# pomonam/LearnablePoolingMethods

Measured on AMD Instinct MI355X. Metric: clips/sec training step, NetVladV1 K=256 300-frame 1152-d, bs=80, 1/2/4/8 GPU, higher is better.
Workload: dtype f32

## Files before the change

### learnablepoolingmethods_amd/csrc/mha_x3.hip

```cpp
#include "lpm_common.h"
#include "operand_format.h"
#include <atomic>
#include <cstdlib>

namespace lpm {

constexpr float MX_LOG2E = 1.4426950408889634f;
constexpr float MX_LN2 = 0.6931471805599453f;
typedef __bf16 mx_bf16x8 __attribute__((ext_vector_type(8)));
typedef __bf16 mx_bf16x2 __attribute__((ext_vector_type(2)));
typedef float mx_f32x2 __attribute__((ext_vector_type(2)));
typedef unsigned mx_u32x4 __attribute__((ext_vector_type(4)));

__device__ __forceinline__ f32x4 mx_mfma(mx_u32x4 a, mx_u32x4 b, f32x4 c) {
    return __builtin_amdgcn_mfma_f32_16x16x32_bf16(__builtin_bit_cast(mx_bf16x8, a), __builtin_bit_cast(mx_bf16x8, b), c, 0, 0, 0);
}
__device__ __forceinline__ void mx_split2(float a, float b, unsigned& hi, unsigned& lo) {
    const mx_f32x2 v = {a, b};
    const mx_bf16x2 h = __builtin_convertvector(v, mx_bf16x2);
    const mx_f32x2 hf = __builtin_convertvector(h, mx_f32x2);
    const mx_bf16x2 l = __builtin_convertvector(v - hf, mx_bf16x2);
    hi = __builtin_bit_cast(unsigned, h);
    lo = __builtin_bit_cast(unsigned, l);
}
// ... 102 lines not shown
        hi[i] = h;
        lo[i] = l;
    }
}
__device__ __forceinline__ void mx_pow2_scale(float amax, float& s, float& inv) {
    const int e = (int)((__float_as_uint(amax) >> 23) & 0xffu);
    const int se = e == 0 ? 127 : min(max(258 - e, 1), 253);
    s = __uint_as_float((unsigned)se << 23);
    inv = __uint_as_float((unsigned)(254 - se) << 23);
}
template <int D>
__device__ __forceinline__ void mx_stage_transposed_h(unsigned char* dst, const float* __restrict__ src, int64_t ld, int b, int L, int LP,
                                                      int hh, int tid, int nt) {
    constexpr int NH = D / 8;
    const int TS = LP * 2 + 16;
    for (int i = tid; i < L * NH; i += nt) {
        const int row = i / NH, hf = i % NH;
        const float* p = src + ((int64_t)b * L + row) * ld + hh * D + 8 * hf;
        const float4 a = *reinterpret_cast<const float4*>(p), c = *reinterpret_cast<const float4*>(p + 4);
        const float v[8] = {a.x, a.y, a.z, a.w, c.x, c.y, c.z, c.w};
        mx_u32x4 hi, lo;
        mx_split8_h(v, 1.f, hi, lo);
        const int pos = (row & ~31) | (((row >> 2) & 3) << 3) | (((row >> 4) & 1) << 2) | (row & 3);
#pragma unroll
        for (int e = 0; e < 8; ++e) {
            const int dd = 8 * hf + e;
            *reinterpret_cast<unsigned short*>(dst + dd * TS + pos * 2) = (unsigned short)(hi[e >> 1] >> ((e & 1) * 16));
            *reinterpret_cast<unsigned short*>(dst + 16 * TS + dd * TS + pos * 2) = (unsigned short)(lo[e >> 1] >> ((e & 1) * 16));
        }
    }
}

__device__ __forceinline__ int mx_perm(int i) { return (i & ~31) | (((i >> 2) & 3) << 3) | (((i >> 4) & 1) << 2) | (i & 3); }

__host__ __device__ constexpr int mx_rowplanes_bytes(int LP, int D) { return (D / 8) * 2 * LP * 16; }
__host__ __device__ constexpr int mx_tstride(int LP) { return LP * 2 + 16; }
__host__ __device__ constexpr int mx_tplanes_bytes(int LP) { return 2 * 16 * mx_tstride(LP); }

template <int D>
__device__ __forceinline__ void mx_stage_rows(unsigned char* dst, const float* __restrict__ src, int64_t ld, int b, int L, int LP,
                                              int hh, float mul, int tid, int nt = 256) {
    constexpr int NH = D / 8;
    for (int i = tid; i < L * NH; i += nt) {
        const int row = i / NH, hf = i % NH;
        const float* p = src + ((int64_t)b * L + row) * ld + hh * D + 8 * hf;
        const float4 a = *reinterpret_cast<const float4*>(p), c = *reinterpret_cast<const float4*>(p + 4);
        const float v[8] = {a.x * mul, a.y * mul, a.z * mul, a.w * mul, c.x * mul, c.y * mul, c.z * mul, c.w * mul};
        mx_u32x4 hi, lo;
        mx_split8(v, hi, lo);
        *reinterpret_cast<mx_u32x4*>(dst + ((0 * NH + hf) * LP + row) * 16) = hi;
        *reinterpret_cast<mx_u32x4*>(dst + ((1 * NH + hf) * LP + row) * 16) = lo;
    }
}
template <int D>
__device__ __forceinline__ void mx_stage_transposed(unsigned char* dst, const float* __restrict__ src, int64_t ld, int b, int L,
                                                    int LP, int hh, int tid, int nt = 256) {
    constexpr int NH = D / 8;
    const int TS = mx_tstride(LP);
    for (int i = tid; i < L * NH; i += nt) {
        const int row = i / NH, hf = i % NH;
        const float* p = src + ((int64_t)b * L + row) * ld + hh * D + 8 * hf;
        const float4 a = *reinterpret_cast<const float4*>(p), c = *reinterpret_cast<const float4*>(p + 4);
        const float v[8] = {a.x, a.y, a.z, a.w, c.x, c.y, c.z, c.w};
        mx_u32x4 hi, lo;
        mx_split8(v, hi, lo);
        const int pos = mx_perm(row);
#pragma unroll
        for (int e = 0; e < 8; ++e) {
            const int dd = 8 * hf + e;
            const unsigned short h16 = (unsigned short)(hi[e >> 1] >> ((e & 1) * 16)), l16 = (unsigned short)(lo[e >> 1] >> ((e & 1) * 16));
            *reinterpret_cast<unsigned short*>(dst + dd * TS + pos * 2) = h16;
            *reinterpret_cast<unsigned short*>(dst + 16 * TS + dd * TS + pos * 2) = l16;
        }
    }
}

template <int D>
__device__ __forceinline__ mx_u32x4 mx_row_frag(const unsigned char* planes, int LP, int t, int l15, int g) {
    const int arr = (D == 16) ? g : ((g == 1) ? 1 : 0);
    return *reinterpret_cast<const mx_u32x4*>(planes + (arr * LP + t * 16 + l15) * 16);
}
template <int D>
__device__ __forceinline__ void mx_col_frags(const mx_u32x4& hi, const mx_u32x4& lo, int g, mx_u32x4& b1, mx_u32x4& b2) {
    const mx_u32x4 z = {0u, 0u, 0u, 0u};
    if (D == 16) {
        b1 = hi;
        b2 = (g < 2) ? lo : z;
    } else {
        b1 = (g < 2) ? hi : ((g == 2) ? lo : z);
        b2 = z;
    }
}

template <int NKT, bool AFFINE, int D, bool RAGGED>
__global__ __launch_bounds__(256) void mha_fwd_x3_kernel(const float* __restrict__ q, const float* __restrict__ k,
                                                         const float* __restrict__ v, int64_t ld, int L, int h, float scale,
                                                         const float* __restrict__ key_scale, const float* __restrict__ key_shift,
                                                         float* __restrict__ o, int64_t ldo, float* __restrict__ lse, int oimg, const MxImg im) {
    static_assert(NKT % 2 == 0, "key tiles come in pairs (32-deep PV reduction)");
    float vmax = 0.f;
    extern __shared__ __attribute__((aligned(16))) unsigned char smem[];
    constexpr int LP = NKT * 16;
    constexpr int NQ = (NKT + 3) / 4;
    const int nkt = (L + 15) >> 4;
    const float qmul = AFFINE ? scale : scale * MX_LOG2E;
    unsigned char* Kp = smem;
    unsigned char* Vt = Kp + mx_rowplanes_bytes(LP, D);
    float* ksc = reinterpret_cast<float*>(Vt + mx_tplanes_bytes(LP));
    float* ksh = ksc + LP;
    const int tid = threadIdx.x, lane = tid & 63, wave = tid >> 6;
    const int l15 = lane & 15, g = lane >> 4;
    const int lid = xcd_remap(blockIdx.x, gridDim.x);
    const int b = lid / h, hh = lid % h;
    const int TS = mx_tstride(LP);

    if (RAGGED || D < 16) {
        for (int i = tid; i < (mx_rowplanes_bytes(LP, D) + mx_tplanes_bytes(LP)) / 16; i += 256)
            reinterpret_cast<mx_u32x4*>(smem)[i] = mx_u32x4{0u, 0u, 0u, 0u};
        __syncthreads();
    }
    if (AFFINE) {
        for (int i = tid; i < LP; i += 256) {
            ksc[i] = (i < L) ? key_scale[i] * MX_LOG2E : 1.f;
            ksh[i] = (i < L) ? key_shift[i] * MX_LOG2E : 0.f;
        }
    }
    mx_stage_rows<D>(Kp, k, ld, b, L, LP, hh, 1.f, tid);
    mx_stage_transposed<D>(Vt, v, ld, b, L, LP, hh, tid);
    __syncthreads();

#pragma unroll 1
    for (int i = 0; i < NQ; ++i) {
        const int qt = wave + 4 * i;
        if (qt >= nkt) break;
        const int qrow = qt * 16 + l15;
        mx_u32x4 qh = {0u, 0u, 0u, 0u}, ql = {0u, 0u, 0u, 0u};
        if (qrow < L) {
            const float* p = q + ((int64_t)b * L + qrow) * ld + hh * D + ((D == 16) ? 8 * (g & 1) : 0);
            const float4 a = *reinterpret_cast<const float4*>(p), c = *reinterpret_cast<const float4*>(p + 4);
            const float qv[8] = {a.x * qmul, a.y * qmul, a.z * qmul, a.w * qmul, c.x * qmul, c.y * qmul, c.z * qmul, c.w * qmul};
            mx_split8(qv, qh, ql);
        }
        mx_u32x4 b1, b2;
        mx_col_frags<D>(qh, ql, g, b1, b2);
        f32x4 p[NKT];
        float m = -INFINITY;
#pragma unroll
        for (int kt = 0; kt < NKT; ++kt) {
            f32x4 acc = {0.f, 0.f, 0.f, 0.f};
            const mx_u32x4 a = mx_row_frag<D>(Kp, LP, kt, l15, g);
            acc = mx_mfma(a, b1, acc);
            if (D == 16) acc = mx_mfma(a, b2, acc);
            if (AFFINE) {
#pragma unroll
                for (int r = 0; r < 4; ++r) acc[r] = fmaf(acc[r], ksc[kt * 16 + 4 * g + r], ksh[kt * 16 + 4 * g + r]);
            }
#pragma unroll
            for (int r = 0; r < 4; ++r) {
                if (RAGGED && kt * 16 + 4 * g + r >= L) acc[r] = -INFINITY;
                m = fmaxf(m, acc[r]);
            }
            p[kt] = acc;
        }
        m = fmaxf(m, __shfl_xor(m, 16, 64));
        m = fmaxf(m, __shfl_xor(m, 32, 64));
        float sum = 0.f;
        f32x4 oa = {0.f, 0.f, 0.f, 0.f}, ob = {0.f, 0.f, 0.f, 0.f};
#pragma unroll
        for (int j = 0; j < NKT / 2; ++j) {
            float e8[8];
#pragma unroll
            for (int r = 0; r < 4; ++r) {
                e8[r] = __builtin_amdgcn_exp2f(p[2 * j][r] - m);
                e8[4 + r] = __builtin_amdgcn_exp2f(p[2 * j + 1][r] - m);
            }
#pragma unroll
            for (int r = 0; r < 8; ++r) sum += e8[r];
            mx_u32x4 ph, pl;
            mx_split8(e8, ph, pl);
            const unsigned char* va = Vt + l15 * TS + (32 * j + 8 * g) * 2;
            const mx_u32x4 vh = *reinterpret_cast<const mx_u32x4*>(va), vl = *reinterpret_cast<const mx_u32x4*>(va + 16 * TS);
            oa = mx_mfma(vh, ph, oa);
            ob = mx_mfma(vh, pl, ob);
            oa = mx_mfma(vl, ph, oa);
        }
        sum += __shfl_xor(sum, 16, 64);
        sum += __shfl_xor(sum, 32, 64);
        const float inv = 1.f / sum;
        if (qrow < L) {
            if (4 * g < D)
                mx_store_act4(o, (int64_t)b * L + qrow, ldo, hh * D + 4 * g, oimg, (oa[0] + ob[0]) * inv, (oa[1] + ob[1]) * inv,
                              (oa[2] + ob[2]) * inv, (oa[3] + ob[3]) * inv, im, vmax);
            if (g == 0) lse[((int64_t)b * h + hh) * L + qrow] = m * MX_LN2 + __logf(sum);
        }
    }
    if (oimg) of_amax_commit(im.oamax, vmax);
}

constexpr int MX_DQ_NT = 512;
template <int NKT, bool AFFINE, int D, bool RAGGED>
__global__ __launch_bounds__(MX_DQ_NT) void mha_bwd_dq_x3_kernel(const float* __restrict__ q, const float* __restrict__ k,
                                                            const float* __restrict__ v, int64_t ld, const float* __restrict__ o,
                                                            const float* __restrict__ dout, int64_t ldo,
                                                            const float* __restrict__ lse, int L, int h, float scale,
                                                            const float* __restrict__ key_scale, const float* __restrict__ key_shift,
                                                            float* __restrict__ dq, int64_t ldd, const float* __restrict__ corr_a,
                                                            const float* __restrict__ corr_b, int img, int oimg, const MxImg im) {
    extern __shared__ __attribute__((aligned(16))) unsigned char smem[];
    float vmax = 0.f;
    constexpr int LP = NKT * 16;
    const int nkt = (L + 15) >> 4;
    const float qmul = AFFINE ? scale : scale * MX_LOG2E;
    unsigned char* Kp = smem;
    unsigned char* Vp = Kp + mx_rowplanes_bytes(LP, D);
    unsigned char* Kt = Vp + mx_rowplanes_bytes(LP, D);
    float* ksc = reinterpret_cast<float*>(Kt + mx_tplanes_bytes(LP));
    float* ksh = ksc + LP;
    float* cas = ksh + LP;
    float* cbs = cas + LP;
    const int tid = threadIdx.x, lane = tid & 63, wave = tid >> 6;
    const int l15 = lane & 15, g = lane >> 4;
    const int lid = xcd_remap(blockIdx.x, gridDim.x);
    const int b = lid / h, hh = lid % h;
    const int TS = mx_tstride(LP);

    if (RAGGED || D < 16) {
        for (int i = tid; i < (2 * mx_rowplanes_bytes(LP, D) + mx_tplanes_bytes(LP)) / 16; i += MX_DQ_NT)
            reinterpret_cast<mx_u32x4*>(smem)[i] = mx_u32x4{0u, 0u, 0u, 0u};
        __syncthreads();
    }
    if (AFFINE) {
        for (int i = tid; i < LP; i += MX_DQ_NT) {
            ksc[i] = (i < L) ? key_scale[i] : 1.f;
            ksh[i] = (i < L) ? key_shift[i] : 0.f;
            cas[i] = (corr_a && i < L) ? corr_a[i] : 0.f;
            cbs[i] = (corr_b && i < L) ? corr_b[i] : 0.f;
        }
    }
    mx_stage_rows<D>(Kp, k, ld, b, L, LP, hh, 1.f, tid, MX_DQ_NT);
    mx_stage_rows<D>(Vp, v, ld, b, L, LP, hh, 1.f, tid, MX_DQ_NT);
    mx_stage_transposed<D>(Kt, k, ld, b, L, LP, hh, tid, MX_DQ_NT);
    __syncthreads();

#pragma unroll 1
    for (int qt = wave; qt < nkt; qt += MX_DQ_NT / 64) {
        const int qrow = qt * 16 + l15;
        const bool qok = qrow < L;
        mx_u32x4 qh = {0u, 0u, 0u, 0u}, ql = qh, gh = qh, gl = qh;
        float dpart = 0.f;
        if (qok) {
            const int c0 = hh * D + ((D == 16) ? 8 * (g & 1) : 0);
            const float* qp = q + ((int64_t)b * L + qrow) * ld + c0;
            const float4 a = *reinterpret_cast<const float4*>(qp), c = *reinterpret_cast<const float4*>(qp + 4);
            const float qv[8] = {a.x * qmul, a.y * qmul, a.z * qmul, a.w * qmul, c.x * qmul, c.y * qmul, c.z * qmul, c.w * qmul};
            mx_split8(qv, qh, ql);
            const int64_t off = ((int64_t)b * L + qrow) * ldo + c0;
            const float4 ga = *reinterpret_cast<const float4*>(dout + off), gc = *reinterpret_cast<const float4*>(dout + off + 4);
            float4 oa, oc;
            mx_load_o8(o, (int64_t)b * L + qrow, ldo, c0, oimg, oa, oc, im);
            const float gv[8] = {ga.x, ga.y, ga.z, ga.w, gc.x, gc.y, gc.z, gc.w};
            mx_split8(gv, gh, gl);
            dpart = ga.x * oa.x + ga.y * oa.y + ga.z * oa.z + ga.w * oa.w + gc.x * oc.x + gc.y * oc.y + gc.z * oc.z + gc.w * oc.w;
        }
        if (D == 16) dpart += __shfl_xor(dpart, 16, 64);
        const float dqv = dpart;
        const float lq = qok ? lse[((int64_t)b * h + hh) * L + qrow] * MX_LOG2E : INFINITY;
        mx_u32x4 qb1, qb2, gb1, gb2;
        mx_col_frags<D>(qh, ql, g, qb1, qb2);
        mx_col_frags<D>(gh, gl, g, gb1, gb2);
        f32x4 dqa = {0.f, 0.f, 0.f, 0.f}, dqb = {0.f, 0.f, 0.f, 0.f};
#pragma unroll 2
        for (int j = 0; j < NKT / 2; ++j) {
            float ds8[8];
#pragma unroll
            for (int t = 0; t < 2; ++t) {
                const int kt = 2 * j + t;
                const mx_u32x4 ka = mx_row_frag<D>(Kp, LP, kt, l15, g), va = mx_row_frag<D>(Vp, LP, kt, l15, g);
                f32x4 st = {0.f, 0.f, 0.f, 0.f}, dp = {0.f, 0.f, 0.f, 0.f};
                st = mx_mfma(ka, qb1, st);
                dp = mx_mfma(va, gb1, dp);
                if (D == 16) {
                    st = mx_mfma(ka, qb2, st);
                    dp = mx_mfma(va, gb2, dp);
                }
                float z[4];
#pragma unroll
                for (int r = 0; r < 4; ++r) {
                    z[r] = st[r];
                    if (AFFINE) z[r] = fmaf(st[r], ksc[kt * 16 + 4 * g + r], ksh[kt * 16 + 4 * g + r]) * MX_LOG2E;
                }
                if (RAGGED) {
#pragma unroll
                    for (int r = 0; r < 4; ++r)
                        if (kt * 16 + 4 * g + r >= L) z[r] = -INFINITY;
                }
#pragma unroll
                for (int r = 0; r < 4; ++r) {
                    const float pr = __builtin_amdgcn_exp2f(z[r] - lq);
                    float dsv = pr * (dp[r] - dqv);
                    if (AFFINE) {
                        const int key = kt * 16 + 4 * g + r;
                        dsv = dsv * ksc[key] - cas[key] - st[r] * cbs[key];
                    }
                    ds8[4 * t + r] = dsv;
                }
            }
            mx_u32x4 dh, dl;
            mx_split8(ds8, dh, dl);
            const unsigned char* kc = Kt + l15 * TS + (32 * j + 8 * g) * 2;
            const mx_u32x4 kh = *reinterpret_cast<const mx_u32x4*>(kc), kl = *reinterpret_cast<const mx_u32x4*>(kc + 16 * TS);
            dqa = mx_mfma(kh, dh, dqa);
            dqb = mx_mfma(kh, dl, dqb);
            dqa = mx_mfma(kl, dh, dqa);
        }
        if (qok && 4 * g < D)
            mx_store_grad4(dq, ((int64_t)b * L + qrow) * ldd + hh * D + 4 * g, img, (dqa[0] + dqb[0]) * scale, (dqa[1] + dqb[1]) * scale,
                           (dqa[2] + dqb[2]) * scale, (dqa[3] + dqb[3]) * scale, im, vmax);
    }
    if (img) of_amax_commit(im.gamax, vmax);
}

#ifndef LPM_DKV_NT_LONG
#define LPM_DKV_NT_LONG 1024
#endif
__host__ __device__ constexpr int mx_dkv_nt(int nkt) { return nkt >= 20 ? LPM_DKV_NT_LONG : 512; }
template <int NKT, bool AFFINE, int D, bool CORR = true>
__global__ __launch_bounds__(mx_dkv_nt(NKT)) void mha_bwd_dkv_x3_kernel(const float* __restrict__ q, const float* __restrict__ k,
                                                             const float* __restrict__ v, int64_t ld, const float* __restrict__ o,
                                                             const float* __restrict__ dout, int64_t ldo,
                                                             const float* __restrict__ lse, int L, int h, float scale,
                                                             const float* __restrict__ key_scale, const float* __restrict__ key_shift,
                                                             float* __restrict__ dk, float* __restrict__ dv, int64_t ldd,
                                                             const float* __restrict__ corr_a, const float* __restrict__ corr_b,
                                                             float* __restrict__ dz_partial, int img, int oimg, const MxImg im) {
    extern __shared__ __attribute__((aligned(16))) unsigned char smem[];
    float vmax = 0.f;
    constexpr int LP = NKT * 16;
    constexpr int MX_DKV_NT = mx_dkv_nt(NKT);
    constexpr int NH = D / 8;
    const int nkt = (L + 15) >> 4;
    const float qmul = AFFINE ? scale : scale * MX_LOG2E;
    unsigned char* Qp = smem;
    unsigned char* Gp = Qp + mx_rowplanes_bytes(LP, D);
    unsigned char* Qt = Gp + mx_rowplanes_bytes(LP, D);
    unsigned char* Gt = Qt + mx_tplanes_bytes(LP);
    float* lses = reinterpret_cast<float*>(Gt + mx_tplanes_bytes(LP));
    float* Dq = lses + LP;
    const bool stats_only = (dk == nullptr);
    const int tid = threadIdx.x, lane = tid & 63, wave = tid >> 6;
    const int l15 = lane & 15, g = lane >> 4;
    const int lid = xcd_remap(blockIdx.x, gridDim.x);
    const int b = lid / h, hh = lid % h;
    const int TS = mx_tstride(LP);

    if (L != LP || D < 16) {
        for (int i = tid; i < (2 * mx_rowplanes_bytes(LP, D) + 2 * mx_tplanes_bytes(LP)) / 16; i += MX_DKV_NT)
            reinterpret_cast<mx_u32x4*>(smem)[i] = mx_u32x4{0u, 0u, 0u, 0u};
    }
    for (int i = tid; i < LP; i += MX_DKV_NT) {
        lses[i] = (i < L) ? lse[((int64_t)b * h + hh) * L + i] * MX_LOG2E : INFINITY;
        Dq[i] = 0.f;
    }
    __syncthreads();
    for (int i0 = 0; i0 < L * NH; i0 += MX_DKV_NT) {
        const int i = i0 + tid;
        float part = 0.f;
        int row = 0;
        if (i < L * NH) {
            row = i / NH;
            const int hf = i % NH;
            const float* qp = q + ((int64_t)b * L + row) * ld + hh * D + 8 * hf;
            const int64_t off = ((int64_t)b * L + row) * ldo + hh * D + 8 * hf;
            const float4 qa = *reinterpret_cast<const float4*>(qp), qc = *reinterpret_cast<const float4*>(qp + 4);
            const float4 ga = *reinterpret_cast<const float4*>(dout + off), gc = *reinterpret_cast<const float4*>(dout + off + 4);
            float4 oa, oc;
            mx_load_o8(o, (int64_t)b * L + row, ldo, hh * D + 8 * hf, oimg, oa, oc, im);
            part = ga.x * oa.x + ga.y * oa.y + ga.z * oa.z + ga.w * oa.w + gc.x * oc.x + gc.y * oc.y + gc.z * oc.z + gc.w * oc.w;
            const float qv[8] = {qa.x * qmul, qa.y * qmul, qa.z * qmul, qa.w * qmul, qc.x * qmul, qc.y * qmul, qc.z * qmul, qc.w * qmul};
            const float gv[8] = {ga.x, ga.y, ga.z, ga.w, gc.x, gc.y, gc.z, gc.w};
            mx_u32x4 qh, ql, gh, gl;
            mx_split8(qv, qh, ql);
            mx_split8(gv, gh, gl);
            *reinterpret_cast<mx_u32x4*>(Qp + ((0 * NH + hf) * LP + row) * 16) = qh;
            *reinterpret_cast<mx_u32x4*>(Qp + ((1 * NH + hf) * LP + row) * 16) = ql;
            *reinterpret_cast<mx_u32x4*>(Gp + ((0 * NH + hf) * LP + row) * 16) = gh;
            *reinterpret_cast<mx_u32x4*>(Gp + ((1 * NH + hf) * LP + row) * 16) = gl;
            const int pos = mx_perm(row);
#pragma unroll
            for (int e = 0; e < 8; ++e) {
                const int dd = 8 * hf + e, sh = (e & 1) * 16;
                *reinterpret_cast<unsigned short*>(Qt + dd * TS + pos * 2) = (unsigned short)(qh[e >> 1] >> sh);
                *reinterpret_cast<unsigned short*>(Qt + 16 * TS + dd * TS + pos * 2) = (unsigned short)(ql[e >> 1] >> sh);
                *reinterpret_cast<unsigned short*>(Gt + dd * TS + pos * 2) = (unsigned short)(gh[e >> 1] >> sh);
                *reinterpret_cast<unsigned short*>(Gt + 16 * TS + dd * TS + pos * 2) = (unsigned short)(gl[e >> 1] >> sh);
            }
        }
        if (NH == 2) part += __shfl_xor(part, 1, 64);
        if (i < L * NH && (i % NH) == 0) Dq[row] = part;
    }
    __syncthreads();

#pragma unroll 1
    for (int kt = wave; kt < nkt; kt += MX_DKV_NT / 64) {
        const int krow = kt * 16 + l15;
        const bool kok = krow < L;
        mx_u32x4 kh = {0u, 0u, 0u, 0u}, kl = kh, vh = kh, vl = kh;
        if (kok) {
            const int64_t off = ((int64_t)b * L + krow) * ld + hh * D + ((D == 16) ? 8 * (g & 1) : 0);
            const float4 ka = *reinterpret_cast<const float4*>(k + off), kc = *reinterpret_cast<const float4*>(k + off + 4);
            const float4 va = *reinterpret_cast<const float4*>(v + off), vc = *reinterpret_cast<const float4*>(v + off + 4);
            const float kv[8] = {ka.x, ka.y, ka.z, ka.w, kc.x, kc.y, kc.z, kc.w};
            const float vv[8] = {va.x, va.y, va.z, va.w, vc.x, vc.y, vc.z, vc.w};
            mx_split8(kv, kh, kl);
            mx_split8(vv, vh, vl);
        }
        mx_u32x4 kb1, kb2, vb1, vb2;
        mx_col_frags<D>(kh, kl, g, kb1, kb2);
        mx_col_frags<D>(vh, vl, g, vb1, vb2);
        const float sck = (key_scale && kok) ? key_scale[krow] : 1.f, shk = (key_shift && kok) ? key_shift[krow] : 0.f;
        const float cak = (corr_a && kok) ? corr_a[krow] : 0.f, cbk = (corr_b && kok) ? corr_b[krow] : 0.f;
        f32x4 dka = {0.f, 0.f, 0.f, 0.f}, dkb = dka, dva = dka, dvb = dka;
        float zs = 0.f, zq = 0.f;
#pragma unroll 2
        for (int j = 0; j < NKT / 2; ++j) {
            float p8[8], ds8[8];
#pragma unroll
            for (int t = 0; t < 2; ++t) {
                const int qt = 2 * j + t;
                const mx_u32x4 qa = mx_row_frag<D>(Qp, LP, qt, l15, g), ga = mx_row_frag<D>(Gp, LP, qt, l15, g);
                f32x4 st = {0.f, 0.f, 0.f, 0.f}, dp = {0.f, 0.f, 0.f, 0.f};
                st = mx_mfma(qa, kb1, st);
                dp = mx_mfma(ga, vb1, dp);
                if (D == 16) {
                    st = mx_mfma(qa, kb2, st);
                    dp = mx_mfma(ga, vb2, dp);
                }
                const float4 lq4v = *reinterpret_cast<const float4*>(lses + qt * 16 + 4 * g);
                const float4 dq4v = *reinterpret_cast<const float4*>(Dq + qt * 16 + 4 * g);
                const float lq4[4] = {lq4v.x, lq4v.y, lq4v.z, lq4v.w}, dq4[4] = {dq4v.x, dq4v.y, dq4v.z, dq4v.w};
#pragma unroll
                for (int r = 0; r < 4; ++r) {
                    const int qr = qt * 16 + 4 * g + r;
                    const float sraw = st[r];
                    float z = sraw;
                    if (AFFINE) z = fmaf(sraw, sck, shk) * MX_LOG2E;
                    if (!kok) z = -INFINITY;
                    const float pr = __builtin_amdgcn_exp2f(z - lq4[r]);
                    const float dz = pr * (dp[r] - dq4[r]);
                    float dsv = dz;
                    if (AFFINE) {
                        zs += dz;
                        zq = fmaf(dz, sraw, zq);
                        if constexpr (CORR) dsv = (qr < L) ? dz * sck - cak - sraw * cbk : 0.f;
                        else dsv = (qr < L) ? dz * sck : 0.f;
                    }
                    p8[4 * t + r] = pr;
                    ds8[4 * t + r] = dsv;
                }
            }
            if (!stats_only) {
                mx_u32x4 ph, pl, dh, dl;
                mx_split8(p8, ph, pl);
                mx_split8(ds8, dh, dl);
                const int offt = l15 * TS + (32 * j + 8 * g) * 2;
                const mx_u32x4 gth = *reinterpret_cast<const mx_u32x4*>(Gt + offt), gtl = *reinterpret_cast<const mx_u32x4*>(Gt + 16 * TS + offt);
                const mx_u32x4 qth = *reinterpret_cast<const mx_u32x4*>(Qt + offt), qtl = *reinterpret_cast<const mx_u32x4*>(Qt + 16 * TS + offt);
                dva = mx_mfma(gth, ph, dva);
                dvb = mx_mfma(gth, pl, dvb);
                dva = mx_mfma(gtl, ph, dva);
                dka = mx_mfma(qth, dh, dka);
                dkb = mx_mfma(qth, dl, dkb);
                dka = mx_mfma(qtl, dh, dka);
            }
        }
        if (!stats_only && kok && 4 * g < D) {
            const int64_t off = ((int64_t)b * L + krow) * ldd + hh * D + 4 * g;
            const float kmul = AFFINE ? 1.f : MX_LN2;
            mx_store_dk4(dk, (int64_t)b * L + krow, ldd, hh * D + 4 * g, img, (dka[0] + dkb[0]) * kmul, (dka[1] + dkb[1]) * kmul, (dka[2] + dkb[2]) * kmul, (dka[3] + dkb[3]) * kmul, im, vmax);
            mx_store_grad4(dv, off, img, dva[0] + dvb[0], dva[1] + dvb[1], dva[2] + dvb[2], dva[3] + dvb[3], im, vmax);
        }
        if (dz_partial) {
            zs += __shfl_xor(zs, 16, 64); zs += __shfl_xor(zs, 32, 64);
            zq += __shfl_xor(zq, 16, 64); zq += __shfl_xor(zq, 32, 64);
            if (g == 0 && kok) {
                float* out = dz_partial + ((int64_t)b * h + hh) * 2 * L;
                out[krow] = zs;
                out[L + krow] = zq;
            }
        }
    }
    if (img) of_amax_commit(im.gamax, vmax);
}

template <int NKT, bool AFFINE, int D, bool RAGGED>
__global__ __launch_bounds__(MX_DQ_NT) void mha_bwd_dq_h_kernel(const float* __restrict__ q, const float* __restrict__ k,
                                                            const float* __restrict__ v, int64_t ld, const float* __restrict__ o,
                                                            const float* __restrict__ dout, int64_t ldo,
                                                            const float* __restrict__ lse, int L, int h, float scale,
                                                            const float* __restrict__ key_scale, const float* __restrict__ key_shift,
                                                            float* __restrict__ dq, int64_t ldd, const float* __restrict__ corr_a,
                                                            const float* __restrict__ corr_b, int img, int oimg, const MxImg im) {
    extern __shared__ __attribute__((aligned(16))) unsigned char smem[];
    float vmax = 0.f;
    constexpr int LP = NKT * 16;
    constexpr int NT = MX_DQ_NT;
    const int nkt = (L + 15) >> 4;
    const float qmul = AFFINE ? scale : scale * MX_LOG2E;
    unsigned char* Kp = smem;
    unsigned char* Vp = Kp + mx_rowplanes_bytes(LP, D);
    unsigned char* Kt = Vp + mx_rowplanes_bytes(LP, D);
    float* ksc = reinterpret_cast<float*>(Kt + mx_tplanes_bytes(LP));
    float* ksh = ksc + LP;
    float* cas = ksh + LP;
    float* cbs = cas + LP;
    const int tid = threadIdx.x, lane = tid & 63, wave = tid >> 6;
    const int l15 = lane & 15, g = lane >> 4;
    const int lid = xcd_remap(blockIdx.x, gridDim.x);
    const int b = lid / h, hh = lid % h;
    const int TS = mx_tstride(LP);
// ... 359 lines not shown
    const int lid = xcd_remap(blockIdx.x, gridDim.x);
    const int b = lid / h, hh = lid % h;
    constexpr int D4 = D / 4;
    float *Qm, *Sq;
    if (moments) {
        Qm = reinterpret_cast<float*>(smem);
        Sq = Qm + D * D;
        for (int i = tid; i < D * D + D; i += 256) Qm[i] = moments[(int64_t)lid * (D * D + D) + i] * (i < D * D ? scale * scale : scale);
        __syncthreads();
    } else {
        float* qs = reinterpret_cast<float*>(smem);
        Qm = qs + (size_t)L * D;
        Sq = Qm + D * D;
        mx_q_moments<D>(q, ld, b, L, hh, scale, qs, Qm, Sq, Sq + D, tid);
    }
    const int c4 = tid % D4;
    float qm[4][D], sq4[4];
#pragma unroll
    for (int u = 0; u < 4; ++u) {
        sq4[u] = Sq[4 * c4 + u];
#pragma unroll
        for (int e = 0; e < D4; ++e) {
            const float4 t = *reinterpret_cast<const float4*>(Qm + (4 * c4 + u) * D + 4 * e);
            qm[u][4 * e] = t.x; qm[u][4 * e + 1] = t.y; qm[u][4 * e + 2] = t.z; qm[u][4 * e + 3] = t.w;
        }
    }
    for (int i = tid; i < L * D4; i += 256) {
        const int row = i / D4;
        const float* kp = k + ((int64_t)b * L + row) * ld + hh * D;
        float kv[D];
#pragma unroll
        for (int e = 0; e < D4; ++e) {
            const float4 t = *reinterpret_cast<const float4*>(kp + 4 * e);
            kv[4 * e] = t.x; kv[4 * e + 1] = t.y; kv[4 * e + 2] = t.z; kv[4 * e + 3] = t.w;
        }
        const float ca = corr_a[row], cb = corr_b[row];
        float* dp = dk + ((int64_t)b * L + row) * ldd + hh * D + 4 * c4;
        float4 g = *reinterpret_cast<float4*>(dp);
        float r[4];
#pragma unroll
        for (int u = 0; u < 4; ++u) {
            float t = 0.f;
#pragma unroll
            for (int e = 0; e < D; ++e) t = fmaf(qm[u][e], kv[e], t);
            r[u] = fmaf(cb, t, ca * sq4[u]);
        }
        g.x -= r[0]; g.y -= r[1]; g.z -= r[2]; g.w -= r[3];
        if (dk_img) mx_store_grad4(dk_img, ((int64_t)b * L + row) * ldi + hh * D + 4 * c4, img, g.x, g.y, g.z, g.w, im, vmax);
        else *reinterpret_cast<float4*>(dp) = g;
    }
    if (dk_img) of_amax_commit(im.gamax, vmax);
}

static inline size_t mx_bwd_dq_lds(int LP, int D) { return (size_t)2 * mx_rowplanes_bytes(LP, D) + mx_tplanes_bytes(LP) + 4 * LP * 4; }
static inline size_t mx_bwd_dkv_lds(int LP, int D) { return (size_t)2 * mx_rowplanes_bytes(LP, D) + 2 * mx_tplanes_bytes(LP) + 2 * LP * 4 + 16; }
static inline size_t mx_fwd_lds(int LP, int D) { return (size_t)mx_rowplanes_bytes(LP, D) + mx_tplanes_bytes(LP) + 2 * LP * 4; }

template <typename KernT>
static int mx_reserve(KernT kern, size_t bytes, const char* what) {
    if (hipFuncSetAttribute((const void*)kern, hipFuncAttributeMaxDynamicSharedMemorySize, (int)bytes) != hipSuccess) {
        (void)hipGetLastError();
        set_error("%s: cannot reserve %zu bytes of LDS", what, bytes);
        return LPM_ERR_LAUNCH;
    }
    return LPM_OK;
}

}

#define LPM_MX_CHECK(name)                                                                                        \
    LPM_REQUIRE(B > 0 && L > 0 && h > 0 && (d == 8 || d == 16) && L <= 512, LPM_ERR_UNSUPPORTED_SHAPE,              \
                name ": need d in {8,16} and L <= 512 (L=%d d=%d)", L, d);                                          \
    LPM_REQUIRE(ld >= (int64_t)h * d && ld % 4 == 0, LPM_ERR_BADARG, name ": bad leading dimension")

static std::atomic<int> g_mha_bwd_terms{lpm::env_first_is("LPM_MHA_BWD_TERMS", '2') ? 2 : 3};
extern "C" int lpm_mha_bwd_set_terms(int terms) {
    if (terms != 2 && terms != 3) return g_mha_bwd_terms.load();
    return g_mha_bwd_terms.exchange(terms);
}

static lpm::MxImg mx_img(const LpmOperandFormat* o_fmt, const LpmOperandFormat* g_fmt) {
    const lpm::OperandFmt fo = lpm::operand_fmt(o_fmt), fg = lpm::operand_fmt(g_fmt);
    return lpm::MxImg{fo.f16, fo.planes, fo.scale, 1.f / fo.scale, fo.amax, fg.f16, fg.planes, fg.scale, fg.amax, 0, 0};
}
static int mx_fwd_launch(const float* q, const float* k, const float* v, int64_t ld, int B, int L, int h, int d, float scale,
                         const float* key_scale, const float* key_shift, float* o, int64_t ldo, float* lse, int oimg,
                         lpm_stream_t stream, const char* what, const LpmOperandFormat* o_fmt = nullptr) {
    using namespace lpm;
    const MxImg im = mx_img(o_fmt, nullptr);
    hipStream_t s = (hipStream_t)stream;
    const int nkt = (L + 15) / 16;
    dim3 grid(B * h);
#define LPM_MX_FWD3(N, AFF, DD, RG)                                                                              \
    do {                                                                                                         \
        auto kern = mha_fwd_x3_kernel<N, AFF, DD, RG>;                                                           \
        const size_t lds = mx_fwd_lds(N * 16, DD);                                                               \
        if (int rc = mx_reserve(kern, lds, what)) return rc;                                                     \
        hipLaunchKernelGGL(kern, grid, dim3(256), lds, s, q, k, v, ld, L, h, scale, key_scale, key_shift, o, ldo, lse, oimg, im); \
    } while (0)
#define LPM_MX_FWD1(N, AFF, RG)        \
    do {                               \
        if (d == 16) LPM_MX_FWD3(N, AFF, 16, RG); \
        else LPM_MX_FWD3(N, AFF, 8, RG); \
    } while (0)
#define LPM_MX_FWD(N)                  \
    do {                               \
        if (key_scale) LPM_MX_FWD1(N, true, true); \
        else if (L == N * 16) LPM_MX_FWD1(N, false, false); \
        else LPM_MX_FWD1(N, false, true); \
// ... 10 lines not shown
}

extern "C" int lpm_mha_fwd_x3(const float* q, const float* k, const float* v, int64_t ld, int B, int L, int h, int d, float scale,
                              const float* key_scale, const float* key_shift, float* o, int64_t ldo, float* lse,
                              lpm_stream_t stream) {
    using namespace lpm;
    LPM_REQUIRE(q && k && v && o && lse, LPM_ERR_BADARG, "lpm_mha_fwd_x3: null pointer");
    LPM_MX_CHECK("lpm_mha_fwd_x3");
    LPM_REQUIRE((key_scale == nullptr) == (key_shift == nullptr), LPM_ERR_BADARG, "lpm_mha_fwd_x3: key_scale/key_shift go together");
    LPM_REQUIRE(ldo >= (int64_t)h * d && ldo % 4 == 0, LPM_ERR_BADARG, "lpm_mha_fwd_x3: bad ldo");
    LPM_REQUIRE((((uintptr_t)q | (uintptr_t)k | (uintptr_t)v | (uintptr_t)o) & 15) == 0, LPM_ERR_BADARG,
                "lpm_mha_fwd_x3: pointers must be 16-byte aligned");
    return mx_fwd_launch(q, k, v, ld, B, L, h, d, scale, key_scale, key_shift, o, ldo, lse, 0, stream, "lpm_mha_fwd_x3");
}

extern "C" int lpm_mha_fwd_x3_image(const float* q, const float* k, const float* v, int64_t ld, int B, int L, int h, int d,
                                    float scale, void* o3, float* lse, lpm_stream_t stream) {
    using namespace lpm;
    LPM_REQUIRE(q && k && v && o3 && lse, LPM_ERR_BADARG, "lpm_mha_fwd_x3_image: null pointer");
    LPM_MX_CHECK("lpm_mha_fwd_x3_image");
    LPM_REQUIRE((((uintptr_t)q | (uintptr_t)k | (uintptr_t)v | (uintptr_t)o3) & 15) == 0, LPM_ERR_BADARG,
                "lpm_mha_fwd_x3_image: pointers must be 16-byte aligned");
    return mx_fwd_launch(q, k, v, ld, B, L, h, d, scale, nullptr, nullptr, (float*)o3, 0, lse, h * d, stream, "lpm_mha_fwd_x3_image");
}
extern "C" int lpm_mha_fwd_x3_image_fmt(const float* q, const float* k, const float* v, int64_t ld, int B, int L, int h, int d,
                                        float scale, void* o3, float* lse, const LpmOperandFormat* o_fmt, lpm_stream_t stream) {
    using namespace lpm;
    LPM_REQUIRE(q && k && v && o3 && lse, LPM_ERR_BADARG, "lpm_mha_fwd_x3_image: null pointer");
    LPM_MX_CHECK("lpm_mha_fwd_x3_image");
    LPM_REQUIRE((((uintptr_t)q | (uintptr_t)k | (uintptr_t)v | (uintptr_t)o3) & 15) == 0, LPM_ERR_BADARG,
                "lpm_mha_fwd_x3_image: pointers must be 16-byte aligned");
    if (const int rc = operand_fmt_check(o_fmt, "lpm_mha_fwd_x3_image")) return rc;
    return mx_fwd_launch(q, k, v, ld, B, L, h, d, scale, nullptr, nullptr, (float*)o3, 0, lse, h * d, stream, "lpm_mha_fwd_x3_image", o_fmt);
}

static int mx_bwd_launch(const float* q, const float* k, const float* v, int64_t ld, const float* o, const float* dout, int64_t ldo,
                         const float* lse, int B, int L, int h, int d, float scale, const float* key_scale, const float* key_shift,
                         float* dq, float* dk, float* dv, int64_t ldd, const float* corr_a, const float* corr_b, float* dz_partial,
                         int img, int oimg, lpm_stream_t stream, const char* what, const LpmOperandFormat* o_fmt = nullptr,
                         const LpmOperandFormat* g_fmt = nullptr, int64_t dk_plain_ld = 0) {
    using namespace lpm;
    MxImg im = mx_img(o_fmt, g_fmt);
    if (dk_plain_ld) {
        im.dk_plain = 1;
        im.dk_ld = dk_plain_ld;
    }
    hipStream_t s = (hipStream_t)stream;
    const int nkt = (L + 15) / 16;
    dim3 grid(B * h);
    const bool h16 = g_mha_bwd_terms.load(std::memory_order_relaxed) == 2 && !corr_a;
#define LPM_MX_BWDH_Q(N, AFF, DD, RG)                                                                                  \
    do {                                                                                                               \
        auto kq = mha_bwd_dq_h_kernel<N, AFF, DD, RG>;                                                                 \
        const size_t lq = mx_bwd_dq_lds(N * 16, DD);                                                                   \
        if (int rc = mx_reserve(kq, lq, what)) return rc;                                                              \
        hipLaunchKernelGGL(kq, grid, dim3(MX_DQ_NT), lq, s, q, k, v, ld, o, dout, ldo, lse, L, h, scale, key_scale, key_shift, \
                           dq, ldd, corr_a, corr_b, img, oimg, im);                                                    \
    } while (0)
#define LPM_MX_BWDH_KV(N, AFF, DD)                                                                                     \
    do {                                                                                                               \
        auto kk = mha_bwd_dkv_h_kernel<N, AFF, DD, false>;                                                             \
        const size_t lk = mx_bwd_dkv_lds(N * 16, DD);                                                                  \
        if (int rc = mx_reserve(kk, lk, what)) return rc;                                                              \
        hipLaunchKernelGGL(kk, grid, dim3(mx_dkv_nt(N)), lk, s, q, k, v, ld, o, dout, ldo, lse, L, h, scale, key_scale, key_shift, \
                           dk, dv, ldd, corr_a, corr_b, dz_partial, img, oimg, im);                                    \
    } while (0)
#define LPM_MX_BWD3(N, AFF, DD, RG)                                                                                    \
    do {                                                                                                               \
        if (h16) {                                                                                                     \
            if (dq) LPM_MX_BWDH_Q(N, AFF, DD, RG);                                                                     \
            if (dk || dz_partial) LPM_MX_BWDH_KV(N, AFF, DD);                                                          \
            break;                                                                                                     \
        }                                                                                                              \
        if (dq) {                                                                                                      \
            auto kq = mha_bwd_dq_x3_kernel<N, AFF, DD, RG>;                                                            \
            const size_t lq = mx_bwd_dq_lds(N * 16, DD);                                                               \
            if (int rc = mx_reserve(kq, lq, what)) return rc;                                                          \
            hipLaunchKernelGGL(kq, grid, dim3(MX_DQ_NT), lq, s, q, k, v, ld, o, dout, ldo, lse, L, h, scale, key_scale, key_shift, dq, \
                               ldd, corr_a, corr_b, img, oimg, im);                                                    \
        }                                                                                                              \
        if (dk || dz_partial) {                                                                                        \
            auto kk = (AFF && !corr_a) ? mha_bwd_dkv_x3_kernel<N, AFF, DD, false> : mha_bwd_dkv_x3_kernel<N, AFF, DD, true>;          \
            const size_t lk = mx_bwd_dkv_lds(N * 16, DD);                                                              \
            if (int rc = mx_reserve(kk, lk, what)) return rc;                                                          \
            hipLaunchKernelGGL(kk, grid, dim3(mx_dkv_nt(N)), lk, s, q, k, v, ld, o, dout, ldo, lse, L, h, scale, key_scale, key_shift, dk, \
                               dv, ldd, corr_a, corr_b, dz_partial, img, oimg, im);                                    \
        }                                                                                                              \
    } while (0)
#define LPM_MX_BWD1(N, AFF, RG)        \
    do {                               \
        if (d == 16) LPM_MX_BWD3(N, AFF, 16, RG); \
        else LPM_MX_BWD3(N, AFF, 8, RG); \
    } while (0)
#define LPM_MX_BWD(N)                  \
    do {                               \
        if (key_scale) LPM_MX_BWD1(N, true, true); \
        else if (L == N * 16) LPM_MX_BWD1(N, false, false); \
        else LPM_MX_BWD1(N, false, true); \
    } while (0)
    if (nkt <= 4) LPM_MX_BWD(4);
    else if (nkt <= 8) LPM_MX_BWD(8);
    else if (nkt <= 16) LPM_MX_BWD(16);
    else if (nkt <= 20) LPM_MX_BWD(20);
    else LPM_MX_BWD(32);
#undef LPM_MX_BWD
#undef LPM_MX_BWD1
#undef LPM_MX_BWD3
#undef LPM_MX_BWDH_Q
#undef LPM_MX_BWDH_KV
    return check_launch(what);
}

extern "C" int lpm_mha_bwd_x3(const float* q, const float* k, const float* v, int64_t ld, const float* o, const float* dout,
                              int64_t ldo, const float* lse, int B, int L, int h, int d, float scale, const float* key_scale,
                              const float* key_shift, float* dq, float* dk, float* dv, int64_t ldd, const float* corr_a,
// ... 114 lines not shown
```

Measured before the change: 12480.

## Replace transposed LDS copies with single XOR-swizzled image read via ds_read_tr16

Operands that were staged in LDS twice, once row-major and once transposed, are now staged once into an XOR-swizzled row image. The transposed fragments for the PV, dQ and dK/dV MFMAs are read with the hardware transpose-load instruction ds_read_tr16_b64. This drops the slow scalar 16-bit transposed stores and roughly halves the LDS footprint of the backward kernels, which may allow more blocks per CU. The risk is bank conflicts or wrong fragment ordering from the new swizzle and transpose-read mapping, and the h-variant kernels keep the old layout.

Measured after the change: 12080. 0.968x the previous value.

```diff
diff --git a/learnablepoolingmethods_amd/csrc/mha_x3.hip b/learnablepoolingmethods_amd/csrc/mha_x3.hip
--- a/learnablepoolingmethods_amd/csrc/mha_x3.hip
+++ b/learnablepoolingmethods_amd/csrc/mha_x3.hip
@@ -178,27 +178,42 @@
         *reinterpret_cast<mx_u32x4*>(dst + ((1 * NH + hf) * LP + row) * 16) = lo;
     }
 }
+__host__ __device__ constexpr int mx_image_bytes(int LP) { return 4 * LP * 16; }
+__device__ __forceinline__ int mx_image_off(int LP, int plane, int hf, int row) { return ((2 * plane + hf) * LP + (row ^ (12 * hf))) * 16; }
 template <int D>
-__device__ __forceinline__ void mx_stage_transposed(unsigned char* dst, const float* __restrict__ src, int64_t ld, int b, int L,
-                                                    int LP, int hh, int tid, int nt = 256) {
+__device__ __forceinline__ void mx_stage_image(unsigned char* dst, const float* __restrict__ src, int64_t ld, int b, int L, int LP,
+                                               int hh, float mul, int tid, int nt) {
     constexpr int NH = D / 8;
-    const int TS = mx_tstride(LP);
     for (int i = tid; i < L * NH; i += nt) {
         const int row = i / NH, hf = i % NH;
         const float* p = src + ((int64_t)b * L + row) * ld + hh * D + 8 * hf;
         const float4 a = *reinterpret_cast<const float4*>(p), c = *reinterpret_cast<const float4*>(p + 4);
-        const float v[8] = {a.x, a.y, a.z, a.w, c.x, c.y, c.z, c.w};
+        const float v[8] = {a.x * mul, a.y * mul, a.z * mul, a.w * mul, c.x * mul, c.y * mul, c.z * mul, c.w * mul};
         mx_u32x4 hi, lo;
         mx_split8(v, hi, lo);
-        const int pos = mx_perm(row);
-#pragma unroll
-        for (int e = 0; e < 8; ++e) {
-            const int dd = 8 * hf + e;
-            const unsigned short h16 = (unsigned short)(hi[e >> 1] >> ((e & 1) * 16)), l16 = (unsigned short)(lo[e >> 1] >> ((e & 1) * 16));
-            *reinterpret_cast<unsigned short*>(dst + dd * TS + pos * 2) = h16;
-            *reinterpret_cast<unsigned short*>(dst + 16 * TS + dd * TS + pos * 2) = l16;
-        }
-    }
+        *reinterpret_cast<mx_u32x4*>(dst + mx_image_off(LP, 0, hf, row)) = hi;
+        *reinterpret_cast<mx_u32x4*>(dst + mx_image_off(LP, 1, hf, row)) = lo;
+    }
+}
+template <int D>
+__device__ __forceinline__ mx_u32x4 mx_image_row_frag(const unsigned char* img, int LP, int t, int l15, int g) {
+    const int plane = (D == 16) ? (g >> 1) : ((g == 1) ? 1 : 0), hf = (D == 16) ? (g & 1) : 0;
+    return *reinterpret_cast<const mx_u32x4*>(img + mx_image_off(LP, plane, hf, t * 16 + l15));
+}
+typedef short mx_i16x4 __attribute__((ext_vector_type(4)));
+typedef __attribute__((address_space(3))) mx_i16x4 mx_lds_i16x4;
+__device__ __forceinline__ mx_u32x4 mx_tr_pair(const unsigned char* a) {
+    mx_lds_i16x4* p = (mx_lds_i16x4*)(a);
+    const mx_i16x4 r0 = __builtin_amdgcn_ds_read_tr16_b64_v4i16(p);
+    const mx_i16x4 r1 = __builtin_amdgcn_ds_read_tr16_b64_v4i16(p + 32);
+    const uint2 u0 = __builtin_bit_cast(uint2, r0), u1 = __builtin_bit_cast(uint2, r1);
+    return mx_u32x4{u0.x, u0.y, u1.x, u1.y};
+}
+__device__ __forceinline__ void mx_tr_frag(const unsigned char* img, int LP, int j, int lane, mx_u32x4& hi, mx_u32x4& lo) {
+    const int g = lane >> 4, q = (lane >> 2) & 3, p = lane & 3;
+    const unsigned char* a = img + mx_image_off(LP, 0, p >> 1, 32 * j + 4 * g + q) + 8 * (p & 1);
+    hi = mx_tr_pair(a);
+    lo = mx_tr_pair(a + 2 * LP * 16);
 }
 
 template <int D>
@@ -231,17 +246,16 @@
     const int nkt = (L + 15) >> 4;
     const float qmul = AFFINE ? scale : scale * MX_LOG2E;
     unsigned char* Kp = smem;
-    unsigned char* Vt = Kp + mx_rowplanes_bytes(LP, D);
-    float* ksc = reinterpret_cast<float*>(Vt + mx_tplanes_bytes(LP));
+    unsigned char* Vi = Kp + mx_rowplanes_bytes(LP, D);
+    float* ksc = reinterpret_cast<float*>(Vi + mx_image_bytes(LP));
     float* ksh = ksc + LP;
     const int tid = threadIdx.x, lane = tid & 63, wave = tid >> 6;
     const int l15 = lane & 15, g = lane >> 4;
     const int lid = xcd_remap(blockIdx.x, gridDim.x);
     const int b = lid / h, hh = lid % h;
-    const int TS = mx_tstride(LP);
 
     if (RAGGED || D < 16) {
-        for (int i = tid; i < (mx_rowplanes_bytes(LP, D) + mx_tplanes_bytes(LP)) / 16; i += 256)
+        for (int i = tid; i < (mx_rowplanes_bytes(LP, D) + mx_image_bytes(LP)) / 16; i += 256)
             reinterpret_cast<mx_u32x4*>(smem)[i] = mx_u32x4{0u, 0u, 0u, 0u};
         __syncthreads();
     }
@@ -252,7 +266,7 @@
         }
     }
     mx_stage_rows<D>(Kp, k, ld, b, L, LP, hh, 1.f, tid);
-    mx_stage_transposed<D>(Vt, v, ld, b, L, LP, hh, tid);
+    mx_stage_image<D>(Vi, v, ld, b, L, LP, hh, 1.f, tid, 256);
     __syncthreads();
 
 #pragma unroll 1
@@ -304,8 +318,8 @@
             for (int r = 0; r < 8; ++r) sum += e8[r];
             mx_u32x4 ph, pl;
             mx_split8(e8, ph, pl);
-            const unsigned char* va = Vt + l15 * TS + (32 * j + 8 * g) * 2;
-            const mx_u32x4 vh = *reinterpret_cast<const mx_u32x4*>(va), vl = *reinterpret_cast<const mx_u32x4*>(va + 16 * TS);
+            mx_u32x4 vh, vl;
+            mx_tr_frag(Vi, LP, j, lane, vh, vl);
             oa = mx_mfma(vh, ph, oa);
             ob = mx_mfma(vh, pl, ob);
             oa = mx_mfma(vl, ph, oa);
@@ -337,10 +351,9 @@
     constexpr int LP = NKT * 16;
     const int nkt = (L + 15) >> 4;
     const float qmul = AFFINE ? scale : scale * MX_LOG2E;
-    unsigned char* Kp = smem;
-    unsigned char* Vp = Kp + mx_rowplanes_bytes(LP, D);
-    unsigned char* Kt = Vp + mx_rowplanes_bytes(LP, D);
-    float* ksc = reinterpret_cast<float*>(Kt + mx_tplanes_bytes(LP));
+    unsigned char* Ki = smem;
+    unsigned char* Vp = Ki + mx_image_bytes(LP);
+    float* ksc = reinterpret_cast<float*>(Vp + mx_rowplanes_bytes(LP, D));
     float* ksh = ksc + LP;
     float* cas = ksh + LP;
     float* cbs = cas + LP;
@@ -348,10 +361,9 @@
     const int l15 = lane & 15, g = lane >> 4;
     const int lid = xcd_remap(blockIdx.x, gridDim.x);
     const int b = lid / h, hh = lid % h;
-    const int TS = mx_tstride(LP);
 
     if (RAGGED || D < 16) {
-        for (int i = tid; i < (2 * mx_rowplanes_bytes(LP, D) + mx_tplanes_bytes(LP)) / 16; i += MX_DQ_NT)
+        for (int i = tid; i < (mx_image_bytes(LP) + mx_rowplanes_bytes(LP, D)) / 16; i += MX_DQ_NT)
             reinterpret_cast<mx_u32x4*>(smem)[i] = mx_u32x4{0u, 0u, 0u, 0u};
         __syncthreads();
     }
@@ -363,9 +375,8 @@
             cbs[i] = (corr_b && i < L) ? corr_b[i] : 0.f;
         }
     }
-    mx_stage_rows<D>(Kp, k, ld, b, L, LP, hh, 1.f, tid, MX_DQ_NT);
+    mx_stage_image<D>(Ki, k, ld, b, L, LP, hh, 1.f, tid, MX_DQ_NT);
     mx_stage_rows<D>(Vp, v, ld, b, L, LP, hh, 1.f, tid, MX_DQ_NT);
-    mx_stage_transposed<D>(Kt, k, ld, b, L, LP, hh, tid, MX_DQ_NT);
     __syncthreads();
 
 #pragma unroll 1
@@ -401,7 +412,7 @@
 #pragma unroll
             for (int t = 0; t < 2; ++t) {
                 const int kt = 2 * j + t;
-                const mx_u32x4 ka = mx_row_frag<D>(Kp, LP, kt, l15, g), va = mx_row_frag<D>(Vp, LP, kt, l15, g);
+                const mx_u32x4 ka = mx_image_row_frag<D>(Ki, LP, kt, l15, g), va = mx_row_frag<D>(Vp, LP, kt, l15, g);
                 f32x4 st = {0.f, 0.f, 0.f, 0.f}, dp = {0.f, 0.f, 0.f, 0.f};
                 st = mx_mfma(ka, qb1, st);
                 dp = mx_mfma(va, gb1, dp);
@@ -433,8 +444,8 @@
             }
             mx_u32x4 dh, dl;
             mx_split8(ds8, dh, dl);
-            const unsigned char* kc = Kt + l15 * TS + (32 * j + 8 * g) * 2;
-            const mx_u32x4 kh = *reinterpret_cast<const mx_u32x4*>(kc), kl = *reinterpret_cast<const mx_u32x4*>(kc + 16 * TS);
+            mx_u32x4 kh, kl;
+            mx_tr_frag(Ki, LP, j, lane, kh, kl);
             dqa = mx_mfma(kh, dh, dqa);
             dqb = mx_mfma(kh, dl, dqb);
             dqa = mx_mfma(kl, dh, dqa);
@@ -466,21 +477,18 @@
     constexpr int NH = D / 8;
     const int nkt = (L + 15) >> 4;
     const float qmul = AFFINE ? scale : scale * MX_LOG2E;
-    unsigned char* Qp = smem;
-    unsigned char* Gp = Qp + mx_rowplanes_bytes(LP, D);
-    unsigned char* Qt = Gp + mx_rowplanes_bytes(LP, D);
-    unsigned char* Gt = Qt + mx_tplanes_bytes(LP);
-    float* lses = reinterpret_cast<float*>(Gt + mx_tplanes_bytes(LP));
+    unsigned char* Qi = smem;
+    unsigned char* Gi = Qi + mx_image_bytes(LP);
+    float* lses = reinterpret_cast<float*>(Gi + mx_image_bytes(LP));
     float* Dq = lses + LP;
     const bool stats_only = (dk == nullptr);
     const int tid = threadIdx.x, lane = tid & 63, wave = tid >> 6;
     const int l15 = lane & 15, g = lane >> 4;
     const int lid = xcd_remap(blockIdx.x, gridDim.x);
     const int b = lid / h, hh = lid % h;
-    const int TS = mx_tstride(LP);
 
     if (L != LP || D < 16) {
-        for (int i = tid; i < (2 * mx_rowplanes_bytes(LP, D) + 2 * mx_tplanes_bytes(LP)) / 16; i += MX_DKV_NT)
+        for (int i = tid; i < 2 * mx_image_bytes(LP) / 16; i += MX_DKV_NT)
             reinterpret_cast<mx_u32x4*>(smem)[i] = mx_u32x4{0u, 0u, 0u, 0u};
     }
     for (int i = tid; i < LP; i += MX_DKV_NT) {
@@ -507,19 +515,10 @@
             mx_u32x4 qh, ql, gh, gl;
             mx_split8(qv, qh, ql);
             mx_split8(gv, gh, gl);
-            *reinterpret_cast<mx_u32x4*>(Qp + ((0 * NH + hf) * LP + row) * 16) = qh;
-            *reinterpret_cast<mx_u32x4*>(Qp + ((1 * NH + hf) * LP + row) * 16) = ql;
-            *reinterpret_cast<mx_u32x4*>(Gp + ((0 * NH + hf) * LP + row) * 16) = gh;
-            *reinterpret_cast<mx_u32x4*>(Gp + ((1 * NH + hf) * LP + row) * 16) = gl;
-            const int pos = mx_perm(row);
-#pragma unroll
-            for (int e = 0; e < 8; ++e) {
-                const int dd = 8 * hf + e, sh = (e & 1) * 16;
-                *reinterpret_cast<unsigned short*>(Qt + dd * TS + pos * 2) = (unsigned short)(qh[e >> 1] >> sh);
-                *reinterpret_cast<unsigned short*>(Qt + 16 * TS + dd * TS + pos * 2) = (unsigned short)(ql[e >> 1] >> sh);
-                *reinterpret_cast<unsigned short*>(Gt + dd * TS + pos * 2) = (unsigned short)(gh[e >> 1] >> sh);
-                *reinterpret_cast<unsigned short*>(Gt + 16 * TS + dd * TS + pos * 2) = (unsigned short)(gl[e >> 1] >> sh);
-            }
+            *reinterpret_cast<mx_u32x4*>(Qi + mx_image_off(LP, 0, hf, row)) = qh;
+            *reinterpret_cast<mx_u32x4*>(Qi + mx_image_off(LP, 1, hf, row)) = ql;
+            *reinterpret_cast<mx_u32x4*>(Gi + mx_image_off(LP, 0, hf, row)) = gh;
+            *reinterpret_cast<mx_u32x4*>(Gi + mx_image_off(LP, 1, hf, row)) = gl;
         }
         if (NH == 2) part += __shfl_xor(part, 1, 64);
         if (i < L * NH && (i % NH) == 0) Dq[row] = part;
@@ -553,7 +552,7 @@
 #pragma unroll
             for (int t = 0; t < 2; ++t) {
                 const int qt = 2 * j + t;
-                const mx_u32x4 qa = mx_row_frag<D>(Qp, LP, qt, l15, g), ga = mx_row_frag<D>(Gp, LP, qt, l15, g);
+                const mx_u32x4 qa = mx_image_row_frag<D>(Qi, LP, qt, l15, g), ga = mx_image_row_frag<D>(Gi, LP, qt, l15, g);
                 f32x4 st = {0.f, 0.f, 0.f, 0.f}, dp = {0.f, 0.f, 0.f, 0.f};
                 st = mx_mfma(qa, kb1, st);
                 dp = mx_mfma(ga, vb1, dp);
@@ -588,9 +587,9 @@
                 mx_u32x4 ph, pl, dh, dl;
                 mx_split8(p8, ph, pl);
                 mx_split8(ds8, dh, dl);
-                const int offt = l15 * TS + (32 * j + 8 * g) * 2;
-                const mx_u32x4 gth = *reinterpret_cast<const mx_u32x4*>(Gt + offt), gtl = *reinterpret_cast<const mx_u32x4*>(Gt + 16 * TS + offt);
-                const mx_u32x4 qth = *reinterpret_cast<const mx_u32x4*>(Qt + offt), qtl = *reinterpret_cast<const mx_u32x4*>(Qt + 16 * TS + offt);
+                mx_u32x4 gth, gtl, qth, qtl;
+                mx_tr_frag(Gi, LP, j, lane, gth, gtl);
+                mx_tr_frag(Qi, LP, j, lane, qth, qtl);
                 dva = mx_mfma(gth, ph, dva);
                 dvb = mx_mfma(gth, pl, dvb);
                 dva = mx_mfma(gtl, ph, dva);
@@ -1056,9 +1055,11 @@
     if (dk_img) of_amax_commit(im.gamax, vmax);
 }
 
-static inline size_t mx_bwd_dq_lds(int LP, int D) { return (size_t)2 * mx_rowplanes_bytes(LP, D) + mx_tplanes_bytes(LP) + 4 * LP * 4; }
-static inline size_t mx_bwd_dkv_lds(int LP, int D) { return (size_t)2 * mx_rowplanes_bytes(LP, D) + 2 * mx_tplanes_bytes(LP) + 2 * LP * 4 + 16; }
-static inline size_t mx_fwd_lds(int LP, int D) { return (size_t)mx_rowplanes_bytes(LP, D) + mx_tplanes_bytes(LP) + 2 * LP * 4; }
+static inline size_t mx_bwd_dq_lds(int LP, int D) { return (size_t)mx_image_bytes(LP) + mx_rowplanes_bytes(LP, D) + 4 * LP * 4; }
+static inline size_t mx_bwd_dkv_lds(int LP, int D) { return (size_t)2 * mx_image_bytes(LP) + 2 * LP * 4 + 16; }
+static inline size_t mx_fwd_lds(int LP, int D) { return (size_t)mx_rowplanes_bytes(LP, D) + mx_image_bytes(LP) + 2 * LP * 4; }
+static inline size_t mx_bwd_dq_h_lds(int LP, int D) { return (size_t)2 * mx_rowplanes_bytes(LP, D) + mx_tplanes_bytes(LP) + 4 * LP * 4; }
+static inline size_t mx_bwd_dkv_h_lds(int LP, int D) { return (size_t)2 * mx_rowplanes_bytes(LP, D) + 2 * mx_tplanes_bytes(LP) + 2 * LP * 4 + 16; }
 
 template <typename KernT>
 static int mx_reserve(KernT kern, size_t bytes, const char* what) {
@@ -1175,7 +1176,7 @@
 #define LPM_MX_BWDH_Q(N, AFF, DD, RG)                                                                                  \
     do {                                                                                                               \
         auto kq = mha_bwd_dq_h_kernel<N, AFF, DD, RG>;                                                                 \
-        const size_t lq = mx_bwd_dq_lds(N * 16, DD);                                                                   \
+        const size_t lq = mx_bwd_dq_h_lds(N * 16, DD);                                                                 \
         if (int rc = mx_reserve(kq, lq, what)) return rc;                                                              \
         hipLaunchKernelGGL(kq, grid, dim3(MX_DQ_NT), lq, s, q, k, v, ld, o, dout, ldo, lse, L, h, scale, key_scale, key_shift, \
                            dq, ldd, corr_a, corr_b, img, oimg, im);                                                    \
@@ -1183,7 +1184,7 @@
 #define LPM_MX_BWDH_KV(N, AFF, DD)                                                                                     \
     do {                                                                                                               \
         auto kk = mha_bwd_dkv_h_kernel<N, AFF, DD, false>;                                                             \
-        const size_t lk = mx_bwd_dkv_lds(N * 16, DD);                                                                  \
+        const size_t lk = mx_bwd_dkv_h_lds(N * 16, DD);                                                                \
         if (int rc = mx_reserve(kk, lk, what)) return rc;                                                              \
         hipLaunchKernelGGL(kk, grid, dim3(mx_dkv_nt(N)), lk, s, q, k, v, ld, o, dout, ldo, lse, L, h, scale, key_scale, key_shift, \
                            dk, dv, ldd, corr_a, corr_b, dz_partial, img, oimg, im);                                    \
```
